# megvii-research/OccDepth

Hardware: AMD Instinct MI355X
Metric: frames/sec forward, SemanticKITTI stereo->256x256x32 voxels (higher is better)
Workload: dtype f32 storage and accumulate; matrix arithmetic as 3x bf16 split (hi + mid + lo of both operands, six v_mfma_f32_32x32x16_bf16 per K step; error vs float64 tested within 1.5x of the exact-fp32 kernels', measured 0.8-1.1x) in the head convolutions (K2s3), the small-volume 3x3x3 convolutions and transpo

## Files before the change

include/occdepth_amd.h:

```cpp
#ifndef OCCDEPTH_AMD_H
#define OCCDEPTH_AMD_H

#include <stdint.h>

#ifdef __cplusplus
extern "C" {
#endif

#define OCCD_OK 0
#define OCCD_EINVAL (-1)
#define OCCD_ELAUNCH (-2)
#define OCCD_ENOMEM (-3)

#define OCCD_MAX_VIEWS 4
#define OCCD_MAX_SCALES 4

#define OCCD_ACT_NONE 0
#define OCCD_ACT_RELU 1
#define OCCD_ACT_SIGMOID 2
#define OCCD_ACT_RELU_PRE 3

#define OCCD_ABI_VERSION 22
int occd_abi_version(void);
const char* occd_strerror(int code);
// ... 184 lines not shown
    const float* ida;
    int64_t* pix;
    uint8_t* fov;
    float* pix_z;
    double vox_origin[3];
    double voxel_size;
    int32_t batch, n_views, X, Y, Z;
    int32_t img_w, img_h;
} occd_vox2pix_args;
int occd_vox2pix(const occd_vox2pix_args* a, void* stream);

int occd_nchw_to_nhwc(const float* in, float* out, int32_t batch, int32_t C,
                      int64_t S, int32_t cs, void* stream);
int occd_nhwc_to_nchw(const float* in, float* out, int32_t batch, int32_t C,
                      int64_t S, int32_t cs, int32_t coff, void* stream);
int occd_softmax_channels(const float* src, float* dst, int64_t rows,
                          int32_t src_cs, int32_t src_coff, int32_t dst_cs,
                          int32_t dst_coff, int32_t n, int32_t dst_pad, void* stream);

int occd_cascade_tail_fwd(const float* part, const float* wn, float* out, int32_t batch, int32_t X,
                          int32_t Y, int32_t Z, int32_t part_cs, int32_t occ_off, int32_t out_cs,
                          int32_t nbr, void* stream);

int occd_affine_act_nchw(const float* x, const float* res, float* y, const float* scale,
                         const float* shift, int32_t batch, int32_t C, int64_t S, int32_t act,
                         float slope, int32_t res_first, void* stream);

int occd_swish_bwd(const float* x, const float* gy, float* gx, int64_t n, void* stream);
int occd_softmax_nchw(const float* x, float* y, int32_t batch, int32_t C, int64_t S, void* stream);
int occd_dwconv2d_nchw(const float* x, const float* w, const float* scale, const float* shift,
                       float* y, int32_t batch, int32_t C, int32_t H, int32_t W, int32_t k,
                       int32_t stride, int32_t pad_top, int32_t pad_left, int32_t Ho, int32_t Wo,
                       int32_t act, void* stream);
int occd_stem_conv3x3_nchw(const float* x, const float* w, const float* scale, const float* shift, float* y,
                           int32_t batch, int32_t H, int32_t W, int32_t cout, int32_t stride, int32_t pad_top,
                           int32_t pad_left, int32_t Ho, int32_t Wo, int32_t act, void* stream);
int occd_upsample_bilinear_cat_nchw(const float* x, const float* skip, float* out, int32_t batch,
                                    int32_t C, int32_t Cskip, int32_t h, int32_t w, int32_t H,
                                    int32_t W, void* stream);
int occd_upsample_bilinear_cat_nhwc(const float* x, const float* skip, float* out, int32_t batch, int32_t C, int32_t Cskip,
                                    int32_t h, int32_t w, int32_t H, int32_t W, void* stream);
int occd_upsample_bilinear_cat_nhwc_rows(const float* x, const float* skip, float* out, int32_t batch, int32_t C, int32_t Cskip,
                                         int32_t h, int32_t w, int32_t H, int32_t W, int32_t out_cs, void* stream);
int occd_upsample_bilinear_nhwc_bwd(const float* gout, float* gx, int32_t batch, int32_t C, int32_t gout_cs, int32_t h,
                                    int32_t w, int32_t H, int32_t W, void* stream);

int occd_upconv_gather_nchw(const float* z, float* out, int32_t batch, int32_t Cout, int32_t h, int32_t w,
                            int32_t H, int32_t W, int64_t z_channel_stride, int64_t z_batch_stride, void* stream);

int occd_upconv_gather_skip_nchw(const float* z, const float* skip, const float* wskip, const float* shift, float* out,
                                 int32_t batch, int32_t Cout, int32_t Cs, int32_t h, int32_t w, int32_t H, int32_t W,
                                 int64_t z_channel_stride, int64_t z_batch_stride, float slope, void* stream);

int occd_wino_input_transform_nchw(const float* x, float* V, int32_t batch, int32_t Cin, int32_t H, int32_t W,
                                   int32_t ty0, int32_t ths, void* stream);
int occd_wino_output_transform_nchw(const float* M, const float* scale, const float* shift, const float* res,
                                    float* y, int32_t batch, int32_t Cout, int32_t H, int32_t W, int32_t ty0,
                                    int32_t ths, int32_t act, float slope, int32_t res_first, void* stream);

int occd_wino_input_transform_cm(const float* x, float* Vt, int32_t batch, int32_t Cin, int32_t H, int32_t W,
                                 int64_t Tp, void* stream);
int occd_wino_output_transform_cm(const float* Mt, const float* scale, const float* shift, const float* res,
                                  float* y, int32_t batch, int32_t Cout, int32_t H, int32_t W, int64_t Tp,
                                  int32_t act, float slope, int32_t res_first, void* stream);

typedef struct occd_wino_args {
    const float* x;
    const float* upk;
    const float* shift;
    const float* res;
    float* y;
    int32_t batch, cin, cout, H, W;
    int32_t act, res_first, tile_hint;
    float slope;
} occd_wino_args;
int64_t occd_wino_packed_floats(int32_t cout, int32_t cin);
int occd_wino_pack_weights(const float* w, const float* scale, float* upk, int32_t cout, int32_t cin, void* stream);
int occd_wino_conv3x3_fwd(const occd_wino_args* a, void* stream);

int64_t occd_wino_packed_f16x2_bytes(int32_t cout, int32_t cin);
int occd_wino_pack_weights_f16x2(const float* w, const float* scale, void* upk, int32_t cout, int32_t cin, void* stream);
int occd_wino_conv3x3_f16x2_fwd(const occd_wino_args* a, void* stream);
int occd_wino_conv3x3_f16x2_fwd_ex(const occd_wino_args* a, int32_t max_workgroups, void* stream);

int occd_dwconv2d_bwd_data_nchw(const float* gy, const float* w, float* dx, int32_t batch, int32_t C, int32_t H,
                                int32_t W, int32_t k, int32_t stride, int32_t pad_top, int32_t pad_left, int32_t Ho,
                                int32_t Wo, void* stream);
int64_t occd_dwconv2d_bwd_weight_workspace_floats(int32_t batch, int32_t C, int32_t k, int32_t Ho, int32_t Wo);
int occd_dwconv2d_bwd_weight_nchw(const float* x, const float* gy, float* dw, float* workspace, int32_t batch, int32_t C,
                                  int32_t H, int32_t W, int32_t k, int32_t stride, int32_t pad_top, int32_t pad_left,
                                  int32_t Ho, int32_t Wo, void* stream);
int32_t occd_dwconv2d_pool_blocks(int32_t Ho, int32_t Wo);
int occd_dwconv2d_pool_nchw(const float* x, const float* w, const float* scale, const float* shift, float* y,
                            float* pool_part, int32_t batch, int32_t C, int32_t H, int32_t W, int32_t k,
                            int32_t stride, int32_t pad_top, int32_t pad_left, int32_t Ho, int32_t Wo,
                            int32_t act, int64_t x_plane_stride, void* stream);
int32_t occd_dwconv2d_set_stage(int32_t form);
int occd_plane_reduce(const float* a, const float* b, float* out, int64_t planes, int64_t S, void* stream);
int occd_se_bwd(const float* gg, const float* gate, const float* sums, const float* r, const float* w_reduce,
                const float* b_reduce, const float* w_expand, float* dz_scratch, float* gm, float* gw_reduce,
                float* gb_reduce, float* gw_expand, float* gb_expand, int32_t batch, int32_t C, int32_t Cr, int64_t S,
                void* stream);
int occd_depthnet_gate(const float* sps, const float* intrins, int64_t intr_stride, float factor, const float* w1,
                       const float* b1, const float* w2, const float* b2, const float* wr, const float* br,
                       const float* we, const float* be, float* gate, int32_t images, int32_t C, void* stream);
int occd_se_gate(const float* pool_part, const float* w_reduce, const float* b_reduce, const float* w_expand,
                 const float* b_expand, float* r_scratch, float* gate, int32_t batch, int32_t C, int32_t Cr,
                 int32_t nblk, int64_t S, void* stream);
int32_t occd_se_gate_set_fused(int32_t on);

int occd_graph_replace_memsets(void* graph);

typedef struct occd_pw_args {
    const float* x;
    const float* wpk;
    const float* shift;
    const float* gate;
    const float* res;
    float* y;
    int64_t N;
    int32_t batch, cin, cout;
    int32_t act, tile_hint;
    float slope;
    int32_t out_nhwc_cs;
} occd_pw_args;
int64_t occd_pw_packed_floats(int32_t cout, int32_t cin);
int occd_pw_pack_weights(const float* w, const float* scale, float* wpk, int32_t cout, int32_t cin, void* stream);
int occd_pw_conv_fwd(const occd_pw_args* a, void* stream);

int occd_argmax_channels(const float* x, int64_t rows, int32_t cs, int32_t coff, int32_t C,
                         const uint16_t* lut, uint16_t* out, void* stream);

#define OCCD_RENDER_MAX_VIEWS 8
typedef struct OccdRenderView {
    float o0[3], ou[3], ov[3];
    float d0[3], du[3], dv[3];
} OccdRenderView;

typedef struct OccdRenderArgs {
    const void* labels;
    const void* target;
    const uint8_t* fov;
    const OccdRenderView* views;
    const uint8_t* palette;
    const uint8_t* background;
    uint8_t* rgb;
    int32_t* hit;
    uint8_t* face;
    float* depth;
    int32_t batch, n_views, H, W;
    int32_t X, Y, Z;
    int32_t label_bytes, target_bytes;
    int32_t n_palette, alpha;
    int32_t view_w[OCCD_RENDER_MAX_VIEWS], view_h[OCCD_RENDER_MAX_VIEWS];
    uint8_t bg_colour[4];
} OccdRenderArgs;
int occd_render_voxels(const OccdRenderArgs* a, void* stream);

typedef struct OccdStereoArgs {
    const float* img;
    uint8_t* gray;
    void* census;
    const float* ida;
    void* workspace;
    uint16_t* S;
    int32_t* d0;
// ... 447 lines not shown
```

occdepth_amd/build.py:

```python
import glob
import os
import shutil
import subprocess
import sys

HERE = os.path.dirname(os.path.abspath(__file__))
CSRC = os.path.join(HERE, "csrc")
SOURCES = ["conv3d_igemm.hip", "conv3d_c32p.hip", "lift.hip", "nchw2d.hip", "loss.hip", "conv3d_wgrad.hip", "conv3d_bf16.hip", "bn.hip", "bneck3d.hip", "rows_gemm.hip", "gemm_x3.hip", "wino2d.hip", "wino_conv2d.hip", "pw_gemm.hip", "se2d.hip", "ipc_allreduce.hip", "graph_fix.hip", "targets.hip", "optim.hip", "render.hip", "stereo.hip", "fuse.hip", "semantic_map.hip", "map_render.hip", "visibility.hip", "ray_metric.hip", "render_loss.hip", "prof.cpp"]
HEADERS = sorted(glob.glob(os.path.join(CSRC, "*.h"))) + [os.path.join(HERE, "..", "include", "occdepth_amd.h")]
LIB = os.path.join(HERE, "libocc_hip.so")
ARCH = "gfx950"
FLAGS = ["-O3", "-std=c++17", "-fPIC"]


def _hipcc():
    exe = shutil.which("hipcc") or "/opt/rocm/bin/hipcc"
    if not os.path.exists(exe):
        raise RuntimeError("hipcc not found: libocc_hip.so cannot be built")
    return exe


def source_digest():
    import hashlib
    h = hashlib.sha256()
    h.update(f"arch={ARCH};flags={' '.join(FLAGS)}".encode())
    for path in [os.path.join(CSRC, s) for s in SOURCES] + HEADERS:
        h.update(os.path.basename(path).encode())
        with open(path, "rb") as f:
            h.update(f.read())
    return h.hexdigest()


STAMP = LIB + ".srchash"


def needs_build():
    if not os.path.exists(LIB) or not os.path.exists(STAMP):
        return True
    with open(STAMP) as f:
        return f.read().strip() != source_digest()


def build(force=False, verbose=True):
    if not force and not needs_build():
        return LIB
    objs = []
    bdir = os.path.join(HERE, "build")
    os.makedirs(bdir, exist_ok=True)
    procs = []
    for s in SOURCES:
        o = os.path.join(bdir, os.path.splitext(s)[0] + ".o")
        cmd = [_hipcc(), f"--offload-arch={ARCH}"] + FLAGS + ["-x", "hip", "-c", os.path.join(CSRC, s), "-o", o]
        if verbose:
            print(" ".join(cmd), flush=True)
        procs.append((subprocess.Popen(cmd), cmd))
        objs.append(o)
    for p, cmd in procs:
        if p.wait() != 0:
            raise RuntimeError("hipcc failed: " + " ".join(cmd))
    cmd = [_hipcc(), f"--offload-arch={ARCH}", "-shared", "-fPIC", "-o", LIB] + objs
    if verbose:
        print(" ".join(cmd), flush=True)
    subprocess.check_call(cmd)
    with open(STAMP, "w") as f:
        f.write(source_digest() + "\n")
    return LIB


if __name__ == "__main__":
    build(force="--force" in sys.argv)
    print(LIB)
```

occdepth_amd/fused.py:

```python
import os

import torch

from . import hip
from .hip import ACT_NONE, ACT_RELU, ACT_RELU_PRE, ACT_SIGMOID, Vox


_warned_eval_with_grad = False


def needs_autograd(module):
    if module.training:
        return True
    if torch.is_grad_enabled():
        global _warned_eval_with_grad
        if not _warned_eval_with_grad:
            _warned_eval_with_grad = True
            import warnings
            warnings.warn("occdepth_amd: eval-mode forward with autograd enabled runs the differentiable ATen path; "
                          "wrap inference in torch.no_grad() to take the HIP eval path", stacklevel=3)
        return True
    return False


def _triple(v):
    return tuple(v) if isinstance(v, (tuple, list)) else (int(v),) * 3


def on_gpu(t):
    return t.is_cuda


def _stamp(*mods):
    key = []
    for m in mods:
        if m is None:
            continue
        for t in list(m.parameters(recurse=False)) + list(m.buffers(recurse=False)):
            key.append((t.data_ptr(), t._version, t.device))
    return tuple(key)


def _bn_affine(bn, cout, device):
    if bn is None:
        return None, torch.zeros(cout, device=device)
    inv = torch.rsqrt(bn.running_var.float() + bn.eps)
    g = bn.weight.float() if bn.weight is not None else torch.ones_like(inv)
    b = bn.bias.float() if bn.bias is not None else torch.zeros_like(inv)
    scale = g * inv
    return scale, b - bn.running_mean.float() * scale


def bn_affine_cached(bn):
    key = _stamp(bn)
    cached = getattr(bn, "_occd_affine", None)
    if cached is None or cached[0] != key:
        scale, shift = _bn_affine(bn, bn.num_features, bn.running_mean.device)
        cached = (key, scale.contiguous(), shift.contiguous())
        bn._occd_affine = cached
    return cached[1], cached[2]


def _same(*values):
    return {v: v for v in values}


_SWITCHES = {
    "WINO_SPLIT": ("OCCDEPTH_WINO_SPLIT", "f16x2", "f16x2", _same("f16x2", "fp32"), "f16x2 or fp32"),
    "BF16X3": ("OCCDEPTH_BF16X3", "head", "0", {"0": False, "": False, "off": False, "false": False, "1": "all", "all": "all",
                                                "on": "all", "true": "all", "head": "head"}, "0, head or 1"),
    "HEAD_SPLIT": ("OCCDEPTH_HEAD_SPLIT", "f16x2", "f16x2", _same("f16x2", "bf16x3"), "f16x2 or bf16x3"),
    "K2B_SPLIT": ("OCCDEPTH_K2B_SPLIT", "f16x2", "f16x2", _same("f16x2", "bf16x3"), "f16x2 or bf16x3"),
    "GEMM_SPLIT": ("OCCDEPTH_GEMM_SPLIT", "f16x2", "f16x2", _same("f16x2", "bf16x3"), "f16x2 or bf16x3"),
}


def _parse(name, v):
    env, _, empty, spellings, expected = _SWITCHES[name]
    v = (v or empty).strip().lower()
    if v not in spellings:
        raise ValueError(f"{env}={v!r}: expected {expected}")
    return spellings[v]


def _from_env(name):
    return _parse(name, os.environ.get(*_SWITCHES[name][:2]))


WINO_SPLIT, BF16X3 = _from_env("WINO_SPLIT"), _from_env("BF16X3")
HEAD_SPLIT, K2B_SPLIT = _from_env("HEAD_SPLIT"), _from_env("K2B_SPLIT")
GEMM_SPLIT = _from_env("GEMM_SPLIT")


def set_wino_split(v):
    global WINO_SPLIT
    WINO_SPLIT = _parse("WINO_SPLIT", v)


def set_bf16x3(on):
    global BF16X3
    BF16X3 = "all" if on is True else _parse("BF16X3", str(on)) if on else False


def set_head_split(v):
    global HEAD_SPLIT
    HEAD_SPLIT = _parse("HEAD_SPLIT", v)


def set_k2b_split(v):
    global K2B_SPLIT
    K2B_SPLIT = _parse("K2B_SPLIT", v)


def set_gemm_split(v):
    global GEMM_SPLIT
    GEMM_SPLIT = _parse("GEMM_SPLIT", v)


def wino_pack(w, scale=None):
    f32 = hip.wino_pack_weights(w, scale)
    if WINO_SPLIT != "f16x2" or not w.is_cuda:
        return f32
    try:
        upk = hip.wino_pack_weights_f16x2(w, scale)
    except ValueError:
        return f32
    upk.f32 = f32
    return upk


def wino_fused_operands(owner, conv, bn):
    key = (_stamp(conv, bn), WINO_SPLIT)
    cache = owner.__dict__.setdefault("_fused_cache", {})
    hit = cache.get(id(conv))
    if hit is None or hit[0] != key:
        scale, shift = bn_affine_cached(bn)
        if conv.bias is not None:
            shift = shift + scale * conv.bias.detach().float()
        hit = (key, wino_pack(conv.weight, scale), shift.contiguous())
        cache[id(conv)] = hit
    return hit[1:]


def _pad_bias(bias, cout):
    out = torch.zeros(hip.round_up(cout, 32), device=bias.device, dtype=torch.float32)
    out[:cout] = bias
    return out


BF16X3_DILATED = os.environ.get("OCCDEPTH_BF16X3_DILATED", "0") == "1"

BF16X3_SMALLVOL = os.environ.get("OCCDEPTH_BF16X3_SMALLVOL", "1") == "1"
SMALLVOL_MAX_VOXELS = 8192
SMALLVOL_KERNELS = ((3, 3, 3), (1, 1, 1)) if os.environ.get("OCCDEPTH_BF16X3_SMALLVOL_K1", "0") == "1" else ((3, 3, 3),)

PHASES_ONE_LAUNCH = os.environ.get("OCCDEPTH_PHASES_ONE_LAUNCH", "1") == "1"
PHASES_X3 = os.environ.get("OCCDEPTH_PHASES_X3", "1") == "1"

K2, K2S3H, K2S3, K2BH, K2B3 = "K2", "K2s3h", "K2s3", "K2bh", "K2b3"
ROUTES = {
    K2: ("f32", "conv3d", {}),
    K2S3H: ("f16x2", "conv3d_f16x2", {}),
    K2S3: ("x3", "conv3d_bf16", {"split3": True}),
    K2BH: ("f16x2", "conv3d_bf16", {"f16x2": True}),
    K2B3: ("x3", "conv3d_bf16", {"split3": True}),
}
_PACKERS = {"f32": lambda w, s, l: hip.pack_weights(w, s, l), "x3": lambda w, s, l: hip.pack_weights_bf16(w, s, l, split3=True),
            "f16x2": lambda w, s, l: hip.pack_weights_f16x2(w, s, l)}


class PackedW:

    def __init__(self, w, scale=None, layout=0):
        self.w, self.scale, self.layout = w, scale, layout
        self.cout, self.cin = (w.shape[1], w.shape[0]) if layout == 2 else (w.shape[0], w.shape[1])
        self.kernel = (1, 1, 1) if layout == 2 else tuple(w.shape[2:])
        self._images = {}
        self._f16x2_ok = None

    def image(self, kind):
        img = self._images.get(kind)
        if img is None:
            img = self._images[kind] = _PACKERS[kind](self.w, self.scale, self.layout)
        return img

    f32, x3 = property(lambda self: self.image("f32")), property(lambda self: self.image("x3"))

    def f16x2_ok(self):
        if self._f16x2_ok is None:
            w, scale = self.w, self.scale
            self._f16x2_ok = w.is_cuda and bool(torch.isfinite(
                w if scale is None else w * scale.view(-1, *([1] * (w.dim() - 1)))).all())
        return self._f16x2_ok


def _aligned(x):
    return x.cs % 8 == 0 and x.coff % 8 == 0


def _small_volume(x, cout, kernel, **kw):
    if kw.get("cin") not in (None, x.C) or x.C < 128 or cout % 128 or not _aligned(x) or x.buf.dtype != torch.float32:
        return False
    pos = kw.get("out_pos")
    if pos is None:
        st, dl, pd = kw.get("stride", (1, 1, 1)), kw.get("dilation", (1, 1, 1)), kw.get("padding", (0, 0, 0))
        pos = tuple((n + 2 * p - d * (k - 1) - 1) // s + 1 for n, p, d, s, k in zip(x.dims, pd, dl, st, kernel))
    return x.batch * pos[0] * pos[1] * pos[2] <= SMALLVOL_MAX_VOXELS and kw.get("tile_hint", 0) == 0


def route(wsrc, x, cout, kernel, out, **kw):
# ... 260 lines not shown
```

occdepth_amd/hip.py:

```python
import collections
import ctypes
import os
from ctypes import c_int32, c_int64, c_void_p

import torch

from . import abi

_HERE = os.path.dirname(os.path.abspath(__file__))
LIB_PATH = os.path.join(_HERE, "libocc_hip.so")

EXPORTS = abi.EXPORTS
ABI_VERSION = abi.ABI_VERSION
MAX_VIEWS = abi.CONSTANTS["OCCD_MAX_VIEWS"]
MAX_SCALES = abi.CONSTANTS["OCCD_MAX_SCALES"]
ACT_NONE = abi.CONSTANTS["OCCD_ACT_NONE"]
ACT_RELU = abi.CONSTANTS["OCCD_ACT_RELU"]
ACT_SIGMOID = abi.CONSTANTS["OCCD_ACT_SIGMOID"]
ACT_RELU_PRE = abi.CONSTANTS["OCCD_ACT_RELU_PRE"]
OPTIM_CHUNK = abi.CONSTANTS["OCCD_OPTIM_CHUNK"]
MAX_REGIONS = abi.CONSTANTS["OCCD_MAX_REGIONS"]

Conv3dArgs = abi.STRUCTS["occd_conv3d_args"]
WgradArgs = abi.STRUCTS["occd_conv3d_wgrad_args"]
# ... 1192 lines not shown
def wino_cm_wins(B, cin, cout, H, W):
    T = B * ((H + 1) // 2) * ((W + 1) // 2)
    return WINO_CM and cin >= WINO_CM_MIN_CIN and cin % 8 == 0 and T >= 4 and \
        16 * -(-cout // 256) * -(-T // 128) >= WINO_CM_MIN_WORKGROUPS


def wino_input_transform_cm(x, Tp=None):
    B, C, H, W = x.shape
    T = B * ((H + 1) // 2) * ((W + 1) // 2)
    Tp = round_up(T, 32) if Tp is None else Tp
    Vt = torch.empty((16, C, Tp), device=x.device, dtype=torch.float32)
    xc = x if x.is_contiguous() else x.contiguous()
    if _PROFILING:
        set_tag("%d @%dx%dx%d" % (C, B, H, W))
    _check(load().occd_wino_input_transform_cm(_f32(xc, "x"), Vt.data_ptr(), B, C, H, W, Tp, _stream()),
           "occd_wino_input_transform_cm")
    return Vt[..., :T]


def wino_output_transform_cm(Mt, shape, scale=None, shift=None, act=None, slope=0.01, res=None, res_first=False):
    B, C, H, W = shape
    T = B * ((H + 1) // 2) * ((W + 1) // 2)
    if Mt.dtype != torch.float32 or tuple(Mt.shape) != (16, C, T) or Mt.stride(2) != 1 or Mt.stride(0) != C * Mt.stride(1):
        raise RuntimeError("wino_output_transform_cm: M^T must be (16, C, T) float32 over dense padded rows")
    y = torch.empty(shape, device=Mt.device, dtype=torch.float32)
    if res is not None and not res.is_contiguous():
        res = res.contiguous()
    if _PROFILING:
        set_tag("%d @%dx%dx%d" % (C, B, H, W))
    if not Mt.is_cuda or Mt.stride(1) < T or Mt.stride(1) % 32:
        raise RuntimeError("wino_output_transform_cm: M^T must be a GPU tensor with rows on a pitch of 32 floats")
    _check(load().occd_wino_output_transform_cm(Mt.data_ptr(), _f32(scale, "scale") if scale is not None else None,
                                                _f32(shift, "shift") if shift is not None else None,
                                                _f32(res, "res") if res is not None else None, _f32(y, "y"), B, C, H, W,
                                                Mt.stride(1), ACT2D[act], float(slope), 1 if res_first else 0, _stream()),
           "occd_wino_output_transform_cm")
    return y


def conv2d_3x3_winograd(x, U, scale=None, shift=None, act=None, slope=0.01, res=None, res_first=False, strip_rows=None,
                        cm=None):
    B, Cin, H, W = x.shape
    th = (H + 1) // 2
    if isinstance(U, WinoCM):
        whole = strip_rows is None or strip_rows >= th
        if GEMM_X3 and whole and x.is_cuda and (wino_cm_wins(B, Cin, U.cout, H, W) if cm is None else cm):
            if U.cin != Cin:
                raise RuntimeError("conv2d_3x3_winograd: the WinoCM operand does not match the input channels")
            Vt = wino_input_transform_cm(x)
            Mt = torch.empty((16, U.cout, Vt.stride(1)), device=x.device, dtype=torch.float32)[..., :Vt.shape[2]]
            gemm_x3(U.image, Vt, out=Mt)
            return wino_output_transform_cm(Mt, (B, U.cout, H, W), scale, shift, act, slope, res, res_first)
        U = U.u()
    cout = U.shape[2]
    if strip_rows is None or strip_rows >= th:
        V = wino_input_transform(x)
        return wino_output_transform(matmul(V, U), (B, cout, H, W), scale, shift, act, slope, res, res_first)
    y = torch.empty((B, cout, H, W), device=x.device, dtype=torch.float32)
    xc = x if x.is_contiguous() else x.contiguous()
    for ty0 in range(0, th, strip_rows):
        ths = min(strip_rows, th - ty0)
        M = matmul(wino_input_transform(xc, ty0, ths), U)
        wino_output_transform(M, tuple(y.shape), scale, shift, act, slope, res, res_first, out=y, ty0=ty0, ths=ths)
    return y


def wino_pack_weights(w, scale=None):
    cout, cin = w.shape[0], w.shape[1]
    if tuple(w.shape[2:]) != (3, 3):
        raise RuntimeError("wino_pack_weights needs a (Cout, Cin, 3, 3) weight")
    n = load().occd_wino_packed_floats(cout, cin)
    if n <= 0:
        raise RuntimeError("occd_wino_packed_floats: bad shape")
    wc = w.detach().float().contiguous()
    upk = torch.empty(n, device=w.device, dtype=torch.float32)
    sc = scale.detach().float().contiguous() if scale is not None else None
    _check(load().occd_wino_pack_weights(_f32(wc, "w"), _f32(sc, "scale") if sc is not None else None,
                                         _f32(upk, "upk"), cout, cin, _stream()), "occd_wino_pack_weights")
    return upk


class WinoF16x2:

    __slots__ = ("image", "cout", "cin", "f32")

    def __init__(self, image, cout, cin, f32=None):
        self.image, self.cout, self.cin, self.f32 = image, cout, cin, f32


_CU_COUNT = {}


def _cu_count(device):
    n = _CU_COUNT.get(device)
    if n is None:
        n = _CU_COUNT[device] = torch.cuda.get_device_properties(device).multi_processor_count
    return n


def wino_f16x2_wins(B, cin, cout, H, W, device=None):
    tiles = B * ((H + 1) // 2) * ((W + 1) // 2)
    return ((cout + 31) // 32) * ((tiles + 127) // 128) >= _cu_count(torch.cuda.current_device() if device is None else device)


def wino_pack_weights_f16x2(w, scale=None):
    cout, cin = w.shape[0], w.shape[1]
    if tuple(w.shape[2:]) != (3, 3):
        raise RuntimeError("wino_pack_weights_f16x2 needs a (Cout, Cin, 3, 3) weight")
    n = load().occd_wino_packed_f16x2_bytes(cout, cin)
    if n <= 0:
        raise RuntimeError("occd_wino_packed_f16x2_bytes: bad shape")
    wc = w.detach().float().contiguous()
    sc = scale.detach().float().contiguous() if scale is not None else None
    image = torch.empty(n, device=w.device, dtype=torch.uint8)
    rc = load().occd_wino_pack_weights_f16x2(_f32(wc, "w"), _f32(sc, "scale") if sc is not None else None,
                                             _ptr(image, "upk"), cout, cin, _stream())
    if rc == -1:
        raise ValueError("wino_pack_weights_f16x2: non-finite weights (keep the float32 image of wino_pack_weights)")
    _check(rc, "occd_wino_pack_weights_f16x2")
    return WinoF16x2(image, cout, cin)


def _parse_wino_persist(value):
    if value not in ("0", "1"):
        raise ValueError("OCCDEPTH_WINO_PERSIST must be 0 or 1, not %r" % (value,))
    return value == "1"


WINO_PERSIST = _parse_wino_persist(os.environ.get("OCCDEPTH_WINO_PERSIST", "0"))


def conv2d_3x3_fused(x, upk, cout, shift=None, act=None, slope=0.01, res=None, res_first=False, tile_hint=0, out=None,
                     max_workgroups=None):
    if not x.is_contiguous():
        x = x.contiguous()
    B, cin, H, W = x.shape
    y = torch.empty((B, cout, H, W), device=x.device, dtype=torch.float32) if out is None else out
    if res is not None and not res.is_contiguous():
        res = res.contiguous()
    if max_workgroups is not None and not isinstance(upk, WinoF16x2):
        raise RuntimeError("max_workgroups is K10h's grid: the operand of this launch is K10's float32 image")
    if isinstance(upk, WinoF16x2) and upk.f32 is not None and not wino_f16x2_wins(B, cin, cout, H, W, x.device):
        upk = upk.f32
    split = isinstance(upk, WinoF16x2)
    a = WinoArgs()
    a.x, a.y = _f32(x, "x"), _f32(y, "y")
    a.upk = _ptr(upk.image, "upk") if split else _f32(upk, "upk")
    a.shift = _f32(shift, "shift") if shift is not None else None
    a.res = _f32(res, "res") if res is not None else None
    a.batch, a.cin, a.cout, a.H, a.W = B, cin, cout, H, W
    a.act, a.res_first, a.tile_hint, a.slope = ACT2D[act], 1 if res_first else 0, int(tile_hint), float(slope)
    if (upk.cout, upk.cin) != (cout, cin) if split else upk.numel() != load().occd_wino_packed_floats(cout, cin):
        raise RuntimeError("packed Winograd weights do not match (cout, cin)")
    if _PROFILING:
        set_tag("%d>%d @%dx%dx%d" % (cin, cout, B, H, W))
    if split:
        if max_workgroups is None:
            max_workgroups = 0 if WINO_PERSIST else -1
        _check(load().occd_wino_conv3x3_f16x2_fwd_ex(ctypes.byref(a), int(max_workgroups), _stream()),
               "occd_wino_conv3x3_f16x2_fwd_ex")
    else:
        _check(load().occd_wino_conv3x3_fwd(ctypes.byref(a), _stream()), "occd_wino_conv3x3_fwd")
    return y


def pw_pack_weights(w, scale=None):
    cout, cin = w.shape[0], w.shape[1]
    n = load().occd_pw_packed_floats(cout, cin)
    if n <= 0 or w.numel() != cout * cin:
        raise RuntimeError("pw_pack_weights needs a (Cout, Cin[, 1, 1]) weight")
    wc = w.detach().float().reshape(cout, cin).contiguous()
    wpk = torch.empty(n, device=w.device, dtype=torch.float32)
    sc = scale.detach().float().contiguous() if scale is not None else None
    _check(load().occd_pw_pack_weights(_f32(wc, "w"), _f32(sc, "scale") if sc is not None else None, _f32(wpk, "wpk"),
                                       cout, cin, _stream()), "occd_pw_pack_weights")
    return wpk


def conv1x1(x, wpk, cout, shift=None, act=None, slope=0.01, gate=None, res=None, tile_hint=0, out=None, nhwc=False):
    if not x.is_contiguous():
        x = x.contiguous()
    B, cin = x.shape[0], x.shape[1]
    sp = tuple(x.shape[2:])
    N = 1
    for d in sp:
        N *= d
    ocs = round_up(cout, 4) if nhwc else 0
    if nhwc:
        y = torch.empty((B,) + sp + (ocs,), device=x.device, dtype=torch.float32)
    else:
        y = torch.empty((B, cout) + sp, device=x.device, dtype=torch.float32) if out is None else out
    if res is not None and not res.is_contiguous():
        res = res.contiguous()
    if gate is not None:
        gate = gate.reshape(B, cin)
        if not gate.is_contiguous():
            gate = gate.contiguous()
    if wpk.numel() != load().occd_pw_packed_floats(cout, cin):
        raise RuntimeError("packed 1x1 weights do not match (cout, cin)")
    a = PwArgs()
    a.x, a.wpk, a.y = _f32(x, "x"), _f32(wpk, "wpk"), _f32(y, "y")
    a.shift = _f32(shift, "shift") if shift is not None else None
    a.gate = _f32(gate, "gate") if gate is not None else None
    a.res = _f32(res, "res") if res is not None else None
    a.N, a.batch, a.cin, a.cout = N, B, cin, cout
    a.act, a.tile_hint, a.slope, a.out_nhwc_cs = ACT2D[act], int(tile_hint), float(slope), ocs
    if _PROFILING:
        set_tag("%d>%d @%dx%d" % (cin, cout, B, N))
    _check(load().occd_pw_conv_fwd(ctypes.byref(a), _stream()), "occd_pw_conv_fwd")
    if nhwc:
        nd = len(sp)
        return y[..., :cout].permute(0, nd + 1, *range(1, nd + 1))
    return y


def dwconv2d_same(x, w, scale, shift, stride, act=None):
    if not x.is_contiguous():
        x = x.contiguous()
    B, C, H, W = x.shape
    k = w.shape[-1]
    Ho, Wo = -(-H // stride), -(-W // stride)
    pad_h = max((Ho - 1) * stride + k - H, 0)
    pad_w = max((Wo - 1) * stride + k - W, 0)
    y = torch.empty((B, C, Ho, Wo), device=x.device, dtype=torch.float32)
    wc = w if w.is_contiguous() else w.contiguous()
    if _PROFILING:
        set_tag("%d k%d s%d @%dx%dx%d" % (C, k, stride, B, H, W))
    _check(load().occd_dwconv2d_nchw(_f32(x, "x"), _f32(wc, "w"), _f32(scale, "scale") if scale is not None else None,
                                     _f32(shift, "shift") if shift is not None else None, _f32(y, "y"), B, C, H, W, k,
                                     stride, pad_h // 2, pad_w // 2, Ho, Wo, ACT2D[act], _stream()),
           "occd_dwconv2d_nchw")
    return y


def depthnet_gate(mlp, se, images, sps=None, intrins=None, factor=1000.0):
    C = mlp.fc2.out_features

    def f(t):
        t = t.detach().float()
# ... 1400 lines not shown
```

Before: 71.39.

## Add direct MFMA 3x3 conv2d kernel with f16x2 split as default path

Adds a direct (non-Winograd) 3x3 convolution kernel. It uses an f16 hi/lo split of both operands on 32x32x16 f16 MFMA, double-buffered weight loads into LDS and a fused BN/activation/residual epilogue. Dispatch picks it by default for eligible shapes (Cin>=64, divisible by 16, enough workgroups to fill the CUs), falling back to Winograd otherwise. The aim is to avoid Winograd transform overhead and its extra memory traffic. The cost is an extra packed weight image per conv and a host sync at pack time.

```diff
diff --git a/include/occdepth_amd.h b/include/occdepth_amd.h
--- a/include/occdepth_amd.h
+++ b/include/occdepth_amd.h
@@ -290,6 +290,10 @@
 int occd_wino_pack_weights_f16x2(const float* w, const float* scale, void* upk, int32_t cout, int32_t cin, void* stream);
 int occd_wino_conv3x3_f16x2_fwd(const occd_wino_args* a, void* stream);
 int occd_wino_conv3x3_f16x2_fwd_ex(const occd_wino_args* a, int32_t max_workgroups, void* stream);
+
+int64_t occd_conv3x3_direct_packed_bytes(int32_t cout, int32_t cin);
+int occd_conv3x3_direct_pack_weights(const float* w, const float* scale, void* image, int32_t cout, int32_t cin, void* stream);
+int occd_conv3x3_direct_fwd(const occd_wino_args* a, void* stream);
 
 int occd_dwconv2d_bwd_data_nchw(const float* gy, const float* w, float* dx, int32_t batch, int32_t C, int32_t H,
                                 int32_t W, int32_t k, int32_t stride, int32_t pad_top, int32_t pad_left, int32_t Ho,
diff --git a/occdepth_amd/build.py b/occdepth_amd/build.py
--- a/occdepth_amd/build.py
+++ b/occdepth_amd/build.py
@@ -6,7 +6,7 @@
 
 HERE = os.path.dirname(os.path.abspath(__file__))
 CSRC = os.path.join(HERE, "csrc")
-SOURCES = ["conv3d_igemm.hip", "conv3d_c32p.hip", "lift.hip", "nchw2d.hip", "loss.hip", "conv3d_wgrad.hip", "conv3d_bf16.hip", "bn.hip", "bneck3d.hip", "rows_gemm.hip", "gemm_x3.hip", "wino2d.hip", "wino_conv2d.hip", "pw_gemm.hip", "se2d.hip", "ipc_allreduce.hip", "graph_fix.hip", "targets.hip", "optim.hip", "render.hip", "stereo.hip", "fuse.hip", "semantic_map.hip", "map_render.hip", "visibility.hip", "ray_metric.hip", "render_loss.hip", "prof.cpp"]
+SOURCES = ["conv3d_igemm.hip", "conv3d_c32p.hip", "lift.hip", "nchw2d.hip", "loss.hip", "conv3d_wgrad.hip", "conv3d_bf16.hip", "bn.hip", "bneck3d.hip", "rows_gemm.hip", "gemm_x3.hip", "wino2d.hip", "wino_conv2d.hip", "conv2d_direct.hip", "pw_gemm.hip", "se2d.hip", "ipc_allreduce.hip", "graph_fix.hip", "targets.hip", "optim.hip", "render.hip", "stereo.hip", "fuse.hip", "semantic_map.hip", "map_render.hip", "visibility.hip", "ray_metric.hip", "render_loss.hip", "prof.cpp"]
 HEADERS = sorted(glob.glob(os.path.join(CSRC, "*.h"))) + [os.path.join(HERE, "..", "include", "occdepth_amd.h")]
 LIB = os.path.join(HERE, "libocc_hip.so")
 ARCH = "gfx950"
diff --git a/occdepth_amd/csrc/conv2d_direct.hip b/occdepth_amd/csrc/conv2d_direct.hip
--- /dev/null
+++ b/occdepth_amd/csrc/conv2d_direct.hip
@@ -0,0 +1,363 @@
+#include <type_traits>
+#include <vector>
+#include "device.h"
+
+namespace {
+
+constexpr int kTH = 8, kTW = 64;
+constexpr int kPR = kTH + 2, kPC = kTW + 2;
+constexpr int kNPIX = kPR * kPC;
+constexpr int kXPlane = 672;
+constexpr int kXBytes = 4 * kXPlane * 16;
+constexpr int kXRounds = (2 * kNPIX + 511) / 512;
+constexpr uint32_t kOutside = 0xFFFFFFF0u;
+
+struct DirP {
+    const float* x;
+    const uint16_t* wpk;
+    const float* fac;
+    const float* shift;
+    const float* res;
+    float* y;
+    int B, Cin, Cout, H, W;
+    int chunks, nblk, ncg, wg_ty, wg_tx, nwg;
+    int act, res_first;
+    float slope;
+    uint32_t wbytes;
+};
+
+template <int NCB>
+struct DirFrag {
+    f16x8 wh[NCB], wlo[NCB], xh[2], xo[2];
+};
+
+template <int NCB>
+__global__ void __launch_bounds__(512, 2) conv3x3_direct_kernel(const DirP p) {
+    constexpr int NREC = 18 * NCB;
+    constexpr int NDMA = (NREC + 7) / 8;
+    constexpr int WBUF = NDMA * 8 * 1024;
+    static_assert(kXBytes + 2 * WBUF <= 160 * 1024, "LDS of a CU");
+    extern __shared__ __attribute__((aligned(16))) float lds[];
+
+    const int tid = threadIdx.x;
+    const int lane = tid & 63;
+    const int wave = __builtin_amdgcn_readfirstlane(tid >> 6);
+    const int li = lane & 31, kk = lane >> 5;
+
+    const uint32_t bid = xcd_remap(blockIdx.x, p.nwg);
+    const int cg = bid % p.ncg;
+    uint32_t t = bid / p.ncg;
+    const int bx = t % p.wg_tx;
+    t /= p.wg_tx;
+    const int by = t % p.wg_ty;
+    const int b = t / p.wg_ty;
+    const int oy0 = by * kTH, ox0 = bx * kTW;
+    const size_t hw = (size_t)p.H * p.W;
+
+    uint32_t voff[kXRounds], xdst[kXRounds];
+#pragma unroll
+    for (int r = 0; r < kXRounds; ++r) {
+        const int e = r * 512 + tid;
+        const int kh = e >= kNPIX ? 1 : 0, pp = e - kh * kNPIX;
+        const int row = pp / kPC, col = pp - row * kPC;
+        const int gy = oy0 - 1 + row, gx = ox0 - 1 + col;
+        const bool ok = e < 2 * kNPIX && (unsigned)gy < (unsigned)p.H && (unsigned)gx < (unsigned)p.W;
+        voff[r] = ok ? (uint32_t)(((size_t)(8 * kh) * hw + (size_t)gy * p.W + gx) * 4) : kOutside;
+        xdst[r] = (uint32_t)((kh * kXPlane + pp) * 4);
+    }
+    const float* const xb = p.x + (size_t)b * p.Cin * hw;
+    float xv[kXRounds][8];
+    auto x_load = [&](int c) {
+#pragma unroll
+        for (int j = 0; j < 8; ++j) {
+            const auto rs = __builtin_amdgcn_make_buffer_rsrc((void*)(xb + (size_t)(c * 16 + j) * hw), 0, (uint32_t)(9 * hw * 4),
+                                                              0x00020000);
+#pragma unroll
+            for (int r = 0; r < kXRounds; ++r)
+                xv[r][j] = __builtin_bit_cast(float, __builtin_amdgcn_raw_buffer_load_b32(rs, voff[r], 0, 0));
+        }
+    };
+    auto x_write = [&]() {
+#pragma unroll
+        for (int r = 0; r < kXRounds; ++r) {
+            u32x4 hi, lo;
+            split2_f16x8((f32x4){xv[r][0], xv[r][1], xv[r][2], xv[r][3]}, (f32x4){xv[r][4], xv[r][5], xv[r][6], xv[r][7]}, hi, lo);
+            if ((r + 1) * 512 <= 2 * kNPIX || r * 512 + tid < 2 * kNPIX) {
+                *(u32x4*)(lds + xdst[r]) = hi;
+                *(u32x4*)(lds + 2 * kXPlane * 4 + xdst[r]) = lo;
+            }
+        }
+    };
+    const auto wrs = __builtin_amdgcn_make_buffer_rsrc((void*)p.wpk, 0, p.wbytes, 0x00020000);
+    auto w_issue = [&](int c, int buf) {
+        const uint32_t src0 = (uint32_t)(((size_t)c * p.nblk + (size_t)cg * NCB) * 18 * 1024) + lane * 16;
+        float* dst = lds + kXBytes / 4 + buf * (WBUF / 4);
+#pragma unroll
+        for (int i = 0; i < NDMA; ++i) {
+            const int rec = i * 8 + wave;
+            __builtin_amdgcn_raw_ptr_buffer_load_lds(wrs, dst + rec * 256, 16, rec < NREC ? src0 + rec * 1024 : kOutside, 0, 0, 0);
+        }
+    };
+
+    using Frag = DirFrag<NCB>;
+    asm volatile("" ::"a"(0.f));
+    f32x16 acc[2][NCB];
+#pragma unroll
+    for (int pb = 0; pb < 2; ++pb)
+#pragma unroll
+        for (int cb = 0; cb < NCB; ++cb)
+#pragma unroll
+            for (int r = 0; r < 16; ++r) acc[pb][cb][r] = 0.f;
+
+    float efc, esh;
+    {
+        const auto ss = __builtin_amdgcn_make_buffer_rsrc((void*)(p.shift != nullptr ? p.shift : p.y), 0,
+                                                          p.shift != nullptr ? (uint32_t)p.Cout * 4u : 0u, 0x00020000);
+        const auto fs = __builtin_amdgcn_make_buffer_rsrc((void*)p.fac, 0, (uint32_t)p.Cout * 4u, 0x00020000);
+        const uint32_t o = tid < 32 * NCB ? (uint32_t)(cg * NCB * 32 + tid) * 4 : kOutside;
+        efc = __builtin_bit_cast(float, __builtin_amdgcn_raw_buffer_load_b32(fs, o, 0, 0));
+        esh = __builtin_bit_cast(float, __builtin_amdgcn_raw_buffer_load_b32(ss, o, 0, 0));
+    }
+    w_issue(0, 0);
+    x_load(0);
+    x_write();
+    __syncthreads();
+
+    const u32x4* const xl = (const u32x4*)lds + (kk * kXPlane + wave * kPC + li);
+    auto run_chunk = [&](auto pass_c, const u32x4* wl) {
+        constexpr int PASS = decltype(pass_c)::value;
+        auto read_tap = [&](int tap, Frag& f) {
+            const int dy = tap / 3, dx = tap % 3;
+#pragma unroll
+            for (int cb = 0; cb < NCB; ++cb) {
+                f.wh[cb] = __builtin_bit_cast(f16x8, wl[((cb * 9 + tap) * 2) * 64]);
+                if (PASS == 0) f.wlo[cb] = __builtin_bit_cast(f16x8, wl[((cb * 9 + tap) * 2 + 1) * 64]);
+            }
+#pragma unroll
+            for (int pb = 0; pb < 2; ++pb) {
+                f.xh[pb] = __builtin_bit_cast(f16x8, xl[dy * kPC + dx + pb * 32]);
+                if (PASS == 0) f.xo[pb] = __builtin_bit_cast(f16x8, xl[2 * kXPlane + dy * kPC + dx + pb * 32]);
+            }
+        };
+        auto mma_tap = [&](const Frag& f) {
+            if (PASS == 0) {
+#pragma unroll
+                for (int pb = 0; pb < 2; ++pb)
+#pragma unroll
+                    for (int cb = 0; cb < NCB; ++cb)
+                        acc[pb][cb] = __builtin_amdgcn_mfma_f32_32x32x16_f16(f.wlo[cb], f.xh[pb], acc[pb][cb], 0, 0, 0);
+                f16x8 ws[NCB];
+#pragma unroll
+                for (int cb = 0; cb < NCB; ++cb) ws[cb] = f.wh[cb] * (_Float16)(1.f / 2048.f);
+#pragma unroll
+                for (int pb = 0; pb < 2; ++pb)
+#pragma unroll
+                    for (int cb = 0; cb < NCB; ++cb)
+                        acc[pb][cb] = __builtin_amdgcn_mfma_f32_32x32x16_f16(ws[cb], f.xo[pb], acc[pb][cb], 0, 0, 0);
+            } else {
+#pragma unroll
+                for (int pb = 0; pb < 2; ++pb)
+#pragma unroll
+                    for (int cb = 0; cb < NCB; ++cb)
+                        acc[pb][cb] = __builtin_amdgcn_mfma_f32_32x32x16_f16(f.wh[cb], f.xh[pb], acc[pb][cb], 0, 0, 0);
+            }
+        };
+        Frag fa, fb;
+        read_tap(0, fa);
+#pragma unroll
+        for (int tap = 0; tap < 9; ++tap) {
+            if (tap + 1 < 9) read_tap(tap + 1, (tap & 1) ? fa : fb);
+            __builtin_amdgcn_sched_barrier(0);
+            mma_tap((tap & 1) ? fb : fa);
+            __builtin_amdgcn_sched_barrier(0);
+        }
+    };
+    auto walk = [&](auto pass_c) {
+        constexpr int PASS = decltype(pass_c)::value;
+        for (int c = 0; c < p.chunks; ++c) {
+            const int it = PASS * p.chunks + c;
+            const bool more = PASS == 0 || c + 1 < p.chunks;
+            if (more) {
+                const int cn = c + 1 < p.chunks ? c + 1 : 0;
+                w_issue(cn, (it + 1) & 1);
+                x_load(cn);
+            }
+            __builtin_amdgcn_sched_barrier(0);
+            run_chunk(pass_c, (const u32x4*)(lds + kXBytes / 4 + (it & 1) * (WBUF / 4)) + lane);
+            __syncthreads();
+            if (more) x_write();
+            __syncthreads();
+        }
+    };
+    walk(std::integral_constant<int, 0>{});
+    walk(std::integral_constant<int, 1>{});
+
+    if (tid < 32 * NCB) {
+        lds[tid] = efc;
+        lds[128 + tid] = esh;
+    }
+    __syncthreads();
+    const int oy = oy0 + wave;
+    uint32_t vo[2];
+#pragma unroll
+    for (int pb = 0; pb < 2; ++pb) {
+        const int ox = ox0 + pb * 32 + li;
+        vo[pb] = oy < p.H && ox < p.W ? (uint32_t)(((size_t)(4 * kk) * hw + (size_t)oy * p.W + ox) * 4) : kOutside;
+    }
+    auto desc = [&](const float* base, int cb, int r) {
+        const int co = (cg * NCB + cb) * 32 + 8 * (r >> 2) + (r & 3);
+        const int rem = p.Cout - co;
+        const uint32_t n = rem <= 0 ? 0u : (uint32_t)((size_t)(rem < 5 ? rem : 5) * hw * 4);
+        return __builtin_amdgcn_make_buffer_rsrc((void*)(rem <= 0 ? p.y : base + ((size_t)b * p.Cout + co) * hw), 0, n, 0x00020000);
+    };
+    auto epilogue = [&](auto has_res) {
+        constexpr bool RES = decltype(has_res)::value;
+        constexpr int NG = 4 * NCB;
+        float ra[8], rb[8];
+        auto res_load = [&](int g, float (&rn)[8]) {
+#pragma unroll
+            for (int i = 0; i < 4; ++i) {
+                const auto rs = desc(p.res, g >> 2, 4 * (g & 3) + i);
+#pragma unroll
+                for (int pb = 0; pb < 2; ++pb)
+                    rn[2 * i + pb] = __builtin_bit_cast(float, __builtin_amdgcn_raw_buffer_load_b32(rs, vo[pb], 0, 0));
+            }
+        };
+        if (RES) res_load(0, ra);
+#pragma unroll
+        for (int g = 0; g < NG; ++g) {
+            const int cb = g >> 2, q = g & 3;
+            float (&cur)[8] = (g & 1) ? rb : ra;
+            if (RES && g + 1 < NG) res_load(g + 1, (g & 1) ? ra : rb);
+            const f32x4 fc4 = *(const f32x4*)(lds + 32 * cb + 8 * q + 4 * kk);
+            const f32x4 sh4 = *(const f32x4*)(lds + 128 + 32 * cb + 8 * q + 4 * kk);
+#pragma unroll
+            for (int i = 0; i < 4; ++i) {
+                const auto ys = desc(p.y, cb, 4 * q + i);
+#pragma unroll
+                for (int pb = 0; pb < 2; ++pb) {
+                    const float rv = RES ? cur[2 * i + pb] : 0.f;
+                    float v = __builtin_fmaf(acc[pb][cb][4 * q + i], fc4[i], sh4[i]);
+                    if (p.res_first) v += rv;
+                    v = act2d_exact(v, p.act, p.slope);
+                    if (!p.res_first) v += rv;
+                    __builtin_amdgcn_raw_buffer_store_b32(__builtin_bit_cast(uint32_t, v), ys, vo[pb], 0, 0);
+                }
+            }
+        }
+    };
+    if (p.res != nullptr) epilogue(std::true_type{});
+    else epilogue(std::false_type{});
+}
+
+__global__ void direct_scale_kernel(const float* __restrict__ w, const float* __restrict__ scale, float* __restrict__ fac,
+                                    int cout, int cin, int nblk) {
+    const int co = blockIdx.x * blockDim.x + threadIdx.x;
+    if (co >= nblk * 32) return;
+    double m = 0.0;
+    bool bad = false;
+    if (co < cout) {
+        const double sc = scale != nullptr ? (double)scale[co] : 1.0;
+        for (int i = 0; i < cin * 9; ++i) {
+            const double v = fabs((double)w[(size_t)co * cin * 9 + i] * sc);
+            if (!(v <= 3.0e38)) bad = true;
+            m = fmax(m, v);
+        }
+    }
+    int e = 0;
+    const bool ok = m > 0.0 && !bad;
+    if (ok) frexp(m, &e);
+    const int k = ok ? min(max(14 - e, -100), 100) : 0;
+    fac[co] = bad ? __builtin_nanf("") : ldexpf(1.f, -(k + kF2XExp));
+}
+
+__global__ void direct_pack_kernel(const float* __restrict__ w, const float* __restrict__ scale, const float* __restrict__ fac,
+                                   uint16_t* __restrict__ wpk, int cout, int cin, int nblk, long total) {
+    const long i = (long)blockIdx.x * blockDim.x + threadIdx.x;
+    if (i >= total) return;
+    const int j = i & 7, lane = (i >> 3) & 63;
+    long t = i >> 9;
+    const int img = t & 1;
+    t >>= 1;
+    const int tap = t % 9; t /= 9;
+    const int blk = t % nblk;
+    const int chunk = (int)(t / nblk);
+    const int co = blk * 32 + (lane & 31), ci = chunk * 16 + (lane >> 5) * 8 + j;
+    float v = 0.f;
+    if (co < cout && ci < cin) {
+        double s = (double)w[((size_t)co * cin + ci) * 9 + tap];
+        if (scale != nullptr) s *= (double)scale[co];
+        v = (float)(s * (double)(ldexpf(1.f, -kF2XExp) / fac[co]));
+    }
+    const _Float16 hi = (_Float16)v;
+    wpk[i] = __builtin_bit_cast(uint16_t, img == 0 ? hi : (_Float16)(v - (float)hi));
+}
+
+template <int NCB>
+int launch_direct(const DirP& p, hipStream_t st) {
+    constexpr size_t lds = kXBytes + 2 * ((18 * NCB + 7) / 8 * 8 * 1024);
+    if (occd::ensure_big_lds(reinterpret_cast<const void*>(conv3x3_direct_kernel<NCB>)) != OCCD_OK) return OCCD_ELAUNCH;
+    hipLaunchKernelGGL((conv3x3_direct_kernel<NCB>), dim3((unsigned)p.nwg), dim3(512), lds, st, p);
+    return occd::check_launch();
+}
+
+int64_t direct_half_count(int32_t cout, int32_t cin) { return (int64_t)(cin / 16) * ((cout + 31) / 32) * 18 * 512; }
+
+}
+
+extern "C" {
+
+int64_t occd_conv3x3_direct_packed_bytes(int32_t cout, int32_t cin) {
+    if (cout < 1 || cin < 1 || cin % 16 != 0) return OCCD_EINVAL;
+    return direct_half_count(cout, cin) * 2 + (int64_t)((cout + 31) / 32) * 32 * 4;
+}
+
+int occd_conv3x3_direct_pack_weights(const float* w, const float* scale, void* image, int32_t cout, int32_t cin, void* stream) {
+    if (w == nullptr || image == nullptr || cout < 1 || cin < 1 || cin % 16 != 0) return OCCD_EINVAL;
+    const int nblk = (cout + 31) / 32;
+    const long total = direct_half_count(cout, cin);
+    if (total * 2 >= 0x7fffffffL) return OCCD_EINVAL;
+    float* fac = reinterpret_cast<float*>(static_cast<uint16_t*>(image) + total);
+    hipLaunchKernelGGL(direct_scale_kernel, dim3((unsigned)nblk), dim3(32), 0, (hipStream_t)stream, w, scale, fac, cout, cin, nblk);
+    hipLaunchKernelGGL(direct_pack_kernel, dim3((unsigned)((total + 255) / 256)), dim3(256), 0, (hipStream_t)stream, w, scale, fac,
+                       static_cast<uint16_t*>(image), cout, cin, nblk, total);
+    const int rc = occd::check_launch();
+    if (rc != OCCD_OK) return rc;
+    std::vector<float> host((size_t)nblk * 32);
+    if (hipMemcpyAsync(host.data(), fac, host.size() * sizeof(float), hipMemcpyDeviceToHost, (hipStream_t)stream) != hipSuccess ||
+        hipStreamSynchronize((hipStream_t)stream) != hipSuccess)
+        return OCCD_ELAUNCH;
+    for (float f : host)
+        if (f != f) return OCCD_EINVAL;
+    return OCCD_OK;
+}
+
+int occd_conv3x3_direct_fwd(const occd_wino_args* a, void* stream) {
+    if (a == nullptr || a->x == nullptr || a->upk == nullptr || a->y == nullptr) return OCCD_EINVAL;
+    if (a->batch < 1 || a->cin < 1 || a->cout < 1 || a->H < 1 || a->W < 1) return OCCD_EINVAL;
+    if (a->cin % 16 != 0 || a->act < 0 || a->act > 3) return OCCD_EINVAL;
+    if (36.0 * a->H * a->W >= 4294967040.0) return OCCD_EINVAL;
+    const int64_t halves = direct_half_count(a->cout, a->cin);
+    if (halves * 2 >= 0x7fffffffL) return OCCD_EINVAL;
+    DirP p{};
+    p.x = a->x; p.shift = a->shift; p.res = a->res; p.y = a->y;
+    p.wpk = reinterpret_cast<const uint16_t*>(a->upk);
+    p.fac = reinterpret_cast<const float*>(p.wpk + halves);
+    p.wbytes = (uint32_t)(halves * 2);
+    p.B = a->batch; p.Cin = a->cin; p.Cout = a->cout; p.H = a->H; p.W = a->W;
+    p.act = a->act; p.res_first = a->res_first; p.slope = a->slope;
+    p.chunks = a->cin / 16;
+    p.nblk = (a->cout + 31) / 32;
+    const int ncb = (p.nblk + 2) / 3 * 3 <= (p.nblk + 1) / 2 * 2 ? 3 : 2;
+    p.ncg = (p.nblk + ncb - 1) / ncb;
+    p.wg_tx = (a->W + kTW - 1) / kTW;
+    p.wg_ty = (a->H + kTH - 1) / kTH;
+    const long nwg = (long)p.ncg * p.wg_tx * p.wg_ty * p.B;
+    if (nwg > 0x7fffffffL) return OCCD_EINVAL;
+    p.nwg = (int)nwg;
+    occd::ProfScope prof("conv3x3_direct_f16x2", (hipStream_t)stream, 2.0 * 9 * p.Cin * p.Cout * (double)p.B * p.H * p.W,
+                         4.0 * p.B * ((double)p.Cin + p.Cout) * p.H * p.W);
+    return ncb == 3 ? launch_direct<3>(p, (hipStream_t)stream) : launch_direct<2>(p, (hipStream_t)stream);
+}
+
+}
diff --git a/occdepth_amd/fused.py b/occdepth_amd/fused.py
--- a/occdepth_amd/fused.py
+++ b/occdepth_amd/fused.py
@@ -72,6 +72,7 @@
     "HEAD_SPLIT": ("OCCDEPTH_HEAD_SPLIT", "f16x2", "f16x2", _same("f16x2", "bf16x3"), "f16x2 or bf16x3"),
     "K2B_SPLIT": ("OCCDEPTH_K2B_SPLIT", "f16x2", "f16x2", _same("f16x2", "bf16x3"), "f16x2 or bf16x3"),
     "GEMM_SPLIT": ("OCCDEPTH_GEMM_SPLIT", "f16x2", "f16x2", _same("f16x2", "bf16x3"), "f16x2 or bf16x3"),
+    "CONV3X3": ("OCCDEPTH_CONV3X3", "direct", "direct", _same("direct", "wino"), "direct or wino"),
 }
 
 
@@ -90,6 +91,7 @@
 WINO_SPLIT, BF16X3 = _from_env("WINO_SPLIT"), _from_env("BF16X3")
 HEAD_SPLIT, K2B_SPLIT = _from_env("HEAD_SPLIT"), _from_env("K2B_SPLIT")
 GEMM_SPLIT = _from_env("GEMM_SPLIT")
+CONV3X3 = _from_env("CONV3X3")
 
 
 def set_wino_split(v):
@@ -115,6 +117,12 @@
 def set_gemm_split(v):
     global GEMM_SPLIT
     GEMM_SPLIT = _parse("GEMM_SPLIT", v)
+
+
+def set_conv3x3(v):
+    global CONV3X3
+    CONV3X3 = _parse("CONV3X3", v)
+    hip.set_conv3x3(CONV3X3)
 
 
 def wino_pack(w, scale=None):
@@ -126,6 +134,8 @@
     except ValueError:
         return f32
     upk.f32 = f32
+    if hip.conv3x3_direct_eligible(w.shape[1], w.shape[0]):
+        upk.direct = hip.conv3x3_direct_pack_weights(w, scale)
     return upk
 
 
diff --git a/occdepth_amd/hip.py b/occdepth_amd/hip.py
--- a/occdepth_amd/hip.py
+++ b/occdepth_amd/hip.py
@@ -1298,10 +1298,10 @@
 
 class WinoF16x2:
 
-    __slots__ = ("image", "cout", "cin", "f32")
-
-    def __init__(self, image, cout, cin, f32=None):
-        self.image, self.cout, self.cin, self.f32 = image, cout, cin, f32
+    __slots__ = ("image", "cout", "cin", "f32", "direct")
+
+    def __init__(self, image, cout, cin, f32=None, direct=None):
+        self.image, self.cout, self.cin, self.f32, self.direct = image, cout, cin, f32, direct
 
 
 _CU_COUNT = {}
@@ -1337,6 +1337,57 @@
     return WinoF16x2(image, cout, cin)
 
 
+def conv3x3_direct_pack_weights(w, scale=None):
+    cout, cin = w.shape[0], w.shape[1]
+    if tuple(w.shape[2:]) != (3, 3):
+        raise RuntimeError("conv3x3_direct_pack_weights needs a (Cout, Cin, 3, 3) weight")
+    n = load().occd_conv3x3_direct_packed_bytes(cout, cin)
+    if n <= 0:
+        raise RuntimeError("occd_conv3x3_direct_packed_bytes: bad shape (Cin must be a multiple of 16)")
+    wc = w.detach().float().contiguous()
+    sc = scale.detach().float().contiguous() if scale is not None else None
+    image = torch.empty(n, device=w.device, dtype=torch.uint8)
+    rc = load().occd_conv3x3_direct_pack_weights(_f32(wc, "w"), _f32(sc, "scale") if sc is not None else None,
+                                                 _ptr(image, "image"), cout, cin, _stream())
+    if rc == -1:
+        raise ValueError("conv3x3_direct_pack_weights: non-finite weights")
+    _check(rc, "occd_conv3x3_direct_pack_weights")
+    return image
+
+
+def _parse_conv3x3(value):
+    value = (value or "direct").strip().lower()
+    if value not in ("direct", "wino"):
+        raise ValueError("OCCDEPTH_CONV3X3=%r: expected direct or wino" % (value,))
+    return value
+
+
+CONV3X3 = _parse_conv3x3(os.environ.get("OCCDEPTH_CONV3X3", "direct"))
+
+
+def set_conv3x3(v):
+    global CONV3X3
+    CONV3X3 = _parse_conv3x3(v)
+
+
+DIRECT_TH, DIRECT_TW = 8, 64
+DIRECT_MIN_CIN = 64
+
+
+def conv3x3_direct_eligible(cin, cout):
+    return cin >= DIRECT_MIN_CIN and cin % 16 == 0
+
+
+def conv3x3_direct_wins(B, cin, cout, H, W, device=None):
+    if not conv3x3_direct_eligible(cin, cout):
+        return False
+    nblk = (cout + 31) // 32
+    if (nblk + 2) // 3 * 3 > (nblk + 1) // 2 * 2:
+        return False
+    wgs = B * ((H + DIRECT_TH - 1) // DIRECT_TH) * ((W + DIRECT_TW - 1) // DIRECT_TW) * ((nblk + 2) // 3)
+    return wgs >= _cu_count(torch.cuda.current_device() if device is None else device)
+
+
 def _parse_wino_persist(value):
     if value not in ("0", "1"):
         raise ValueError("OCCDEPTH_WINO_PERSIST must be 0 or 1, not %r" % (value,))
@@ -1347,7 +1398,9 @@
 
 
 def conv2d_3x3_fused(x, upk, cout, shift=None, act=None, slope=0.01, res=None, res_first=False, tile_hint=0, out=None,
-                     max_workgroups=None):
+                     max_workgroups=None, kernel=None):
+    if kernel not in (None, "direct", "wino"):
+        raise ValueError("kernel must be None, 'direct' or 'wino', not %r" % (kernel,))
     if not x.is_contiguous():
         x = x.contiguous()
     B, cin, H, W = x.shape
@@ -1356,12 +1409,19 @@
         res = res.contiguous()
     if max_workgroups is not None and not isinstance(upk, WinoF16x2):
         raise RuntimeError("max_workgroups is K10h's grid: the operand of this launch is K10's float32 image")
-    if isinstance(upk, WinoF16x2) and upk.f32 is not None and not wino_f16x2_wins(B, cin, cout, H, W, x.device):
+    if kernel == "direct":
+        if not isinstance(upk, WinoF16x2) or upk.direct is None or max_workgroups is not None:
+            raise RuntimeError("kernel='direct' needs a WinoF16x2 that carries K10d's image, and no max_workgroups")
+        direct = True
+    else:
+        direct = (kernel is None and isinstance(upk, WinoF16x2) and upk.direct is not None and CONV3X3 == "direct"
+                  and max_workgroups is None and x.is_cuda and conv3x3_direct_wins(B, cin, cout, H, W, x.device))
+    if not direct and isinstance(upk, WinoF16x2) and upk.f32 is not None and not wino_f16x2_wins(B, cin, cout, H, W, x.device):
         upk = upk.f32
     split = isinstance(upk, WinoF16x2)
     a = WinoArgs()
     a.x, a.y = _f32(x, "x"), _f32(y, "y")
-    a.upk = _ptr(upk.image, "upk") if split else _f32(upk, "upk")
+    a.upk = _ptr(upk.direct if direct else upk.image, "upk") if split else _f32(upk, "upk")
     a.shift = _f32(shift, "shift") if shift is not None else None
     a.res = _f32(res, "res") if res is not None else None
     a.batch, a.cin, a.cout, a.H, a.W = B, cin, cout, H, W
@@ -1370,7 +1430,9 @@
         raise RuntimeError("packed Winograd weights do not match (cout, cin)")
     if _PROFILING:
         set_tag("%d>%d @%dx%dx%d" % (cin, cout, B, H, W))
-    if split:
+    if direct:
+        _check(load().occd_conv3x3_direct_fwd(ctypes.byref(a), _stream()), "occd_conv3x3_direct_fwd")
+    elif split:
         if max_workgroups is None:
             max_workgroups = 0 if WINO_PERSIST else -1
         _check(load().occd_wino_conv3x3_f16x2_fwd_ex(ctypes.byref(a), int(max_workgroups), _stream()),
```

Result: slower. 70.26 (-1.6%).
